# Breakthrough/PySceneDetect

Measured on NVIDIA H100. Metric: frames/sec scored (1080p, ContentDetector), higher is better.
Workload: dtype u8

## Files before the change

### pyscenedetect_b200/csrc/engine.cu

```cuda
#include <math.h>
#include <stdarg.h>
#include <string.h>

#include <vector>

#include "psd_common.cuh"

namespace psd {

static thread_local char g_err[512] = "";
std::atomic<uint64_t> g_launches{0};

void set_error(const char* fmt, ...) {
    va_list ap;
    va_start(ap, fmt);
    vsnprintf(g_err, sizeof(g_err), fmt, ap);
    va_end(ap);
}

static void build_taps(int src, int dst, std::vector<int32_t>& ofs, std::vector<int16_t>& coef) {
    ofs.resize(dst);
    coef.resize(2 * (size_t)dst);
    const double scale = (double)src / (double)dst;
    for (int d = 0; d < dst; ++d) {
// ... 161 lines not shown
    e->last_n = n;
    PSD_CUDA(cudaEventRecord(t1, st));
    e->ev_total.push_back({t0, t1});
    return PSD_OK;
}

extern "C" {

int psd_abi_version(void) { return PSD_ABI_VERSION; }
const char* psd_version(void) { return "psd_b200 0.1.0 (sm_90a)"; }
const char* psd_last_error(void) { return g_err; }
uint64_t psd_launch_count(void) { return g_launches.load(); }

int psd_device_count(void) {
    int n = 0;
    if (cudaGetDeviceCount(&n) != cudaSuccess) { cudaGetLastError(); return 0; }
    return n;
}

int psd_device_info(int device, char* name_out, size_t name_cap, int* cc_major, int* cc_minor,
                    int* sm_count, uint64_t* total_mem) {
    cudaDeviceProp p{};
    PSD_CUDA(cudaGetDeviceProperties(&p, device));
    if (name_out && name_cap) { strncpy(name_out, p.name, name_cap - 1); name_out[name_cap - 1] = 0; }
    if (cc_major) *cc_major = p.major;
    if (cc_minor) *cc_minor = p.minor;
    if (sm_count) *sm_count = p.multiProcessorCount;
    if (total_mem) *total_mem = (uint64_t)p.totalGlobalMem;
    return PSD_OK;
}

int psd_device_pci_bus_id(int device, char* out, size_t cap) {
    PSD_REQUIRE(out && cap >= 16, "psd_device_pci_bus_id: buffer too small");
    PSD_CUDA(cudaDeviceGetPCIBusId(out, (int)cap, device));
    return PSD_OK;
}

int psd_host_alloc(size_t bytes, void** out) {
    PSD_REQUIRE(out && bytes > 0, "psd_host_alloc: bad args");
    PSD_CUDA(cudaHostAlloc(out, bytes, cudaHostAllocDefault));
    return PSD_OK;
}
int psd_host_free(void* p) {
    if (p) PSD_CUDA(cudaFreeHost(p));
    return PSD_OK;
}
int psd_device_alloc(int device, size_t bytes, void** out) {
    PSD_REQUIRE(out && bytes > 0, "psd_device_alloc: bad args");
    PSD_CUDA(cudaSetDevice(device));
    PSD_CUDA(cudaMalloc(out, bytes));
    return PSD_OK;
}
int psd_device_free(int device, void* p) {
    PSD_CUDA(cudaSetDevice(device));
    if (p) PSD_CUDA(cudaFree(p));
    return PSD_OK;
}
int psd_memcpy_h2d(int device, void* dst, const void* src, size_t bytes) {
    PSD_CUDA(cudaSetDevice(device));
    PSD_CUDA(cudaMemcpy(dst, src, bytes, cudaMemcpyHostToDevice));
    return PSD_OK;
}
int psd_memcpy_d2h(int device, void* dst, const void* src, size_t bytes) {
    PSD_CUDA(cudaSetDevice(device));
    PSD_CUDA(cudaMemcpy(dst, src, bytes, cudaMemcpyDeviceToHost));
    return PSD_OK;
}

void psd_engine_destroy(psd_engine* e) {
    if (!e) return;
    cudaSetDevice(e->device);
    if (e->compute_stream) cudaStreamSynchronize(e->compute_stream);
    if (e->copy_stream) cudaStreamSynchronize(e->copy_stream);
    for (int s = 0; s < 2; ++s) {
        if (e->pinned[s]) cudaFreeHost(e->pinned[s]);
        if (e->dev_stage[s]) cudaFree(e->dev_stage[s]);
        if (e->slot_free[s]) cudaEventDestroy(e->slot_free[s]);
        if (e->h2d_done[s]) cudaEventDestroy(e->h2d_done[s]);
    }
    cudaFree(e->small); cudaFree(e->d_xofs); cudaFree(e->d_xa); cudaFree(e->d_yofs); cudaFree(e->d_ya);
    cudaFree(e->carry); cudaFree(e->d_sums); cudaFree(e->d_yhist); cudaFree(e->d_hash);
    hash_plan_destroy(&e->hash);
    cudaFree(e->eb.vplane); cudaFree(e->eb.vhist); cudaFree(e->eb.thresholds); cudaFree(e->eb.cand);
    cudaFree(e->eb.tmp); cudaFree(e->eb.bits_in); cudaFree(e->eb.bits_dil); cudaFree(e->eb.bits_hdil);
    cudaFree(e->eb.carry_bits); cudaFree(e->eb.dirty); cudaFree(e->eb.hyst_flags);
    for (cudaEvent_t ev : e->ev_pool) cudaEventDestroy(ev);
    if (e->copy_stream) cudaStreamDestroy(e->copy_stream);
    if (e->compute_stream) cudaStreamDestroy(e->compute_stream);
    delete e;
}

#define ENG_CUDA(expr)                                                                          \
    do {                                                                                        \
        cudaError_t _e = (expr);                                                                \
        if (_e != cudaSuccess) {                                                                \
            psd::set_error("%s failed: %s (%s:%d)", #expr, cudaGetErrorString(_e), __FILE__,    \
                           __LINE__);                                                           \
            psd_engine_destroy(e);                                                              \
            return (_e == cudaErrorMemoryAllocation) ? PSD_ERR_OOM : PSD_ERR_CUDA;              \
        }                                                                                       \
    } while (0)

int psd_engine_create(const psd_config* cfg, psd_engine** out) {
    PSD_REQUIRE(cfg && out, "psd_engine_create: null argument");
    PSD_REQUIRE(cfg->struct_size == (int32_t)sizeof(psd_config), "psd_config.struct_size mismatch");
    PSD_REQUIRE(cfg->src_width > 0 && cfg->src_height > 0 && cfg->width > 0 && cfg->height > 0,
                "frame sizes must be positive");
    PSD_REQUIRE((int64_t)cfg->src_width * cfg->src_height < (1LL << 30), "frame too large");
    PSD_REQUIRE(cfg->features != 0 && (cfg->features & ~31u) == 0, "bad feature mask 0x%x", cfg->features);
    PSD_REQUIRE(cfg->max_batch >= 1 && cfg->max_batch <= 4096, "max_batch must be in [1,4096]");
    PSD_REQUIRE(cfg->edge_kernel_size == 0 || (cfg->edge_kernel_size >= 3 && (cfg->edge_kernel_size & 1)),
                "kernel_size must be odd integer >= 3");
    PSD_REQUIRE(cfg->flags == 0, "psd_config.flags must be 0 (no flags are defined), got 0x%x", cfg->flags);
    int ndev = 0;
    if (cudaGetDeviceCount(&ndev) != cudaSuccess || ndev == 0) {
        cudaGetLastError();
        set_error("no CUDA device visible (this engine has no CPU fallback)");
        return PSD_ERR_NODEVICE;
    }
    PSD_REQUIRE(cfg->device >= 0 && cfg->device < ndev, "device %d out of range (%d visible)", cfg->device, ndev);
    cudaDeviceProp prop{};
    PSD_CUDA(cudaGetDeviceProperties(&prop, cfg->device));
    if (prop.major != 9 || prop.minor != 0) {
        set_error("device %d is sm_%d%d; this library is built for sm_90a only", cfg->device, prop.major,
                  prop.minor);
        return PSD_ERR_NODEVICE;
    }
    PSD_CUDA(cudaSetDevice(cfg->device));
    psd_engine* e = new (std::nothrow) psd_engine();
    if (!e) { set_error("out of host memory"); return PSD_ERR_OOM; }
    e->cfg = *cfg;
    e->device = cfg->device;
    e->sw = cfg->src_width; e->sh = cfg->src_height; e->W = cfg->width; e->H = cfg->height;
    e->resize = (e->sw != e->W) || (e->sh != e->H);
    e->P = (int64_t)e->W * e->H;
    e->frame_bytes = e->P * 3;
    e->small_stride = (e->frame_bytes + 15) & ~(int64_t)15;
    e->src_frame_bytes = (int64_t)e->sw * e->sh * 3;
    e->features = cfg->features | ((cfg->features & PSD_F_EDGES) ? PSD_F_HSV : 0);
    e->max_batch = cfg->max_batch;
    if (e->features & PSD_F_EDGES) {
        int k = cfg->edge_kernel_size;
        if (k == 0) {
            k = 4 + (int)nearbyint(sqrt((double)e->W * (double)e->H) / 192.0);
            if ((k & 1) == 0) k += 1;
        }
        if (edge_dilate_check(e->W, k) != PSD_OK) {
            psd_engine_destroy(e);
            return PSD_ERR_INVALID;
        }
        e->ksize = k;
    }
    if (e->features & PSD_F_HASH) {
        int rc = hash_plan_create(&e->hash, e->W, e->H, cfg->hash_size ? cfg->hash_size : 8,
                                  cfg->hash_lowpass ? cfg->hash_lowpass : 2, e->max_batch);
        if (rc) { psd_engine_destroy(e); return rc; }
    }
    ENG_CUDA(cudaStreamCreateWithFlags(&e->copy_stream, cudaStreamNonBlocking));
    ENG_CUDA(cudaStreamCreateWithFlags(&e->compute_stream, cudaStreamNonBlocking));
    for (int s = 0; s < 2; ++s) {
        ENG_CUDA(cudaEventCreateWithFlags(&e->slot_free[s], cudaEventDisableTiming));
        ENG_CUDA(cudaEventCreateWithFlags(&e->h2d_done[s], cudaEventDisableTiming));
    }
    ENG_CUDA(cudaMalloc(&e->carry, (size_t)e->frame_bytes));
    if (e->resize || e->frame_bytes % 16 != 0)
        ENG_CUDA(cudaMalloc(&e->small, (size_t)e->small_stride * e->max_batch));
    if (e->resize) {
        std::vector<int32_t> xo, yo; std::vector<int16_t> xa, ya;
        build_taps(e->sw, e->W, xo, xa);
        build_taps(e->sh, e->H, yo, ya);
        ENG_CUDA(cudaMalloc(&e->d_xofs, xo.size() * 4)); ENG_CUDA(cudaMalloc(&e->d_xa, xa.size() * 2));
        ENG_CUDA(cudaMalloc(&e->d_yofs, yo.size() * 4)); ENG_CUDA(cudaMalloc(&e->d_ya, ya.size() * 2));
        ENG_CUDA(cudaMemcpy(e->d_xofs, xo.data(), xo.size() * 4, cudaMemcpyHostToDevice));
        ENG_CUDA(cudaMemcpy(e->d_xa, xa.data(), xa.size() * 2, cudaMemcpyHostToDevice));
        ENG_CUDA(cudaMemcpy(e->d_yofs, yo.data(), yo.size() * 4, cudaMemcpyHostToDevice));
        ENG_CUDA(cudaMemcpy(e->d_ya, ya.data(), ya.size() * 2, cudaMemcpyHostToDevice));
    }
    if (e->features & PSD_F_EDGES) {
        const size_t plane = (size_t)e->P * e->max_batch;
        ENG_CUDA(cudaMalloc(&e->eb.vplane, plane));
        const size_t words = (size_t)e->H * ((e->W + 31) / 32);
        const size_t tiled = (size_t)edge_tile_words(e->W, e->H) * 4 * e->max_batch;
        ENG_CUDA(cudaMalloc(&e->eb.cand, tiled));
        ENG_CUDA(cudaMalloc(&e->eb.bits_in, tiled));
        ENG_CUDA(cudaMemset(e->eb.cand, 0, tiled));
        ENG_CUDA(cudaMemset(e->eb.bits_in, 0, tiled));
        ENG_CUDA(cudaMalloc(&e->eb.tmp, (size_t)e->P));
        ENG_CUDA(cudaMalloc(&e->eb.bits_dil, words * 4 * e->max_batch));
        if (edge_dilate_separable(e->ksize)) ENG_CUDA(cudaMalloc(&e->eb.bits_hdil, words * 4 * e->max_batch));
        ENG_CUDA(cudaMalloc(&e->eb.carry_bits, words * 4));
        ENG_CUDA(cudaMalloc(&e->eb.vhist, (size_t)e->max_batch * 256 * 4));
        ENG_CUDA(cudaMalloc(&e->eb.thresholds, (size_t)e->max_batch * 2 * 4));
        ENG_CUDA(cudaMalloc(&e->eb.hyst_flags, 64));
        const size_t n_tiles = (size_t)e->max_batch * ((e->W + 63) / 64) * ((e->H + 31) / 32);
        ENG_CUDA(cudaMalloc(&e->eb.dirty, 2 * n_tiles));
    }
    {
        int rc = ensure_capacity(e, 4096);
        if (rc) { psd_engine_destroy(e); return rc; }
    }
    *out = e;
    return PSD_OK;
}

int psd_engine_reset(psd_engine* e) {
    PSD_REQUIRE(e, "null engine");
    PSD_CUDA(cudaSetDevice(e->device));
    PSD_CUDA(cudaStreamSynchronize(e->copy_stream));
    PSD_CUDA(cudaStreamSynchronize(e->compute_stream));
    e->n_frames = 0;
    e->have_carry = false;
    e->halo_scored = false;
    e->last_n = 0;
    e->ev_next = 0; e->ev_score.clear(); e->ev_total.clear();
    return PSD_OK;
}

static int ensure_staging(psd_engine* e) {
    for (int s = 0; s < 2; ++s) {
        if (!e->dev_stage[s]) PSD_CUDA(cudaMalloc(&e->dev_stage[s], (size_t)e->src_frame_bytes * e->max_batch));
    }
    return PSD_OK;
}
static int ensure_pinned(psd_engine* e) {
    for (int s = 0; s < 2; ++s) {
        if (!e->pinned[s])
            PSD_CUDA(cudaHostAlloc((void**)&e->pinned[s], (size_t)e->src_frame_bytes * e->max_batch,
                                   cudaHostAllocDefault));
    }
    return PSD_OK;
}

static int stage_host(psd_engine* e, const uint8_t* bgr, int64_t n, int64_t frame_stride,
                      int64_t row_pitch, uint32_t flags, int slot) {
    const int64_t tight_row = (int64_t)e->sw * 3;
    PSD_CUDA(cudaEventSynchronize(e->slot_free[slot]));
    const uint8_t* src = bgr;
    int64_t fs = frame_stride, rp = row_pitch;
    if (!(flags & PSD_SUBMIT_PINNED)) {
        int rc = ensure_pinned(e);
        if (rc) return rc;
        uint8_t* dst = e->pinned[slot];
        if (rp == tight_row && fs == e->src_frame_bytes) {
            memcpy(dst, bgr, (size_t)(n * e->src_frame_bytes));
        } else {
            for (int64_t f = 0; f < n; ++f)
                for (int y = 0; y < e->sh; ++y)
                    memcpy(dst + f * e->src_frame_bytes + (int64_t)y * tight_row,
                           bgr + f * frame_stride + (int64_t)y * row_pitch, (size_t)tight_row);
        }
        src = dst; fs = e->src_frame_bytes; rp = tight_row;
    }
    if (rp == tight_row && fs == e->src_frame_bytes) {
        PSD_CUDA(cudaMemcpyAsync(e->dev_stage[slot], src, (size_t)(n * e->src_frame_bytes),
                                 cudaMemcpyHostToDevice, e->copy_stream));
    } else {
        for (int64_t f = 0; f < n; ++f)
            PSD_CUDA(cudaMemcpy2DAsync(e->dev_stage[slot] + f * e->src_frame_bytes, (size_t)tight_row,
                                       src + f * fs, (size_t)rp, (size_t)tight_row, (size_t)e->sh,
                                       cudaMemcpyHostToDevice, e->copy_stream));
    }
    PSD_CUDA(cudaEventRecord(e->h2d_done[slot], e->copy_stream));
    PSD_CUDA(cudaStreamWaitEvent(e->compute_stream, e->h2d_done[slot], 0));
    return PSD_OK;
}

int psd_engine_set_halo_device(psd_engine* e, const void* dptr) {
    PSD_REQUIRE(e && dptr, "psd_engine_set_halo_device: null argument");
    PSD_REQUIRE(e->n_frames == 0, "halo must be set before the first frame is submitted");
    PSD_CUDA(cudaSetDevice(e->device));
    e->have_carry = false;
    int rc = run_batch(e, (const uint8_t*)dptr, e->src_frame_bytes, 1, 0, true);
    if (rc) return rc;
    e->halo_scored = true;
    return PSD_OK;
}

int psd_engine_set_halo_host(psd_engine* e, const uint8_t* bgr, int64_t row_pitch) {
    PSD_REQUIRE(e && bgr, "psd_engine_set_halo_host: null argument");
    PSD_REQUIRE(e->n_frames == 0, "halo must be set before the first frame is submitted");
    PSD_REQUIRE(row_pitch >= (int64_t)e->sw * 3, "row_pitch smaller than a row");
    PSD_CUDA(cudaSetDevice(e->device));
    int rc = ensure_staging(e);
    if (rc) return rc;
    const int slot = e->next_slot;
    e->next_slot ^= 1;
    rc = stage_host(e, bgr, 1, row_pitch * e->sh, row_pitch, 0, slot);
    if (rc) return rc;
    rc = psd_engine_set_halo_device(e, e->dev_stage[slot]);
    if (rc) return rc;
    PSD_CUDA(cudaEventRecord(e->slot_free[slot], e->compute_stream));
    return PSD_OK;
}

int psd_engine_submit_device(psd_engine* e, const void* dptr, int64_t n, int64_t frame_stride) {
    PSD_REQUIRE(e && dptr, "psd_engine_submit_device: null argument");
    PSD_REQUIRE(n >= 0, "negative frame count");
    PSD_REQUIRE(frame_stride >= e->src_frame_bytes, "frame_stride smaller than a frame");
    if (n == 0) return PSD_OK;
    PSD_CUDA(cudaSetDevice(e->device));
    int rc = ensure_capacity(e, e->n_frames + n + 1);
    if (rc) return rc;
    const uint8_t* p = (const uint8_t*)dptr;
    int64_t done = 0;
    while (done < n) {
        const int64_t b = (n - done < e->max_batch) ? (n - done) : e->max_batch;
        rc = run_batch(e, p + done * frame_stride, frame_stride, b, e->n_frames + 1, false);
        if (rc) return rc;
        e->n_frames += b;
        done += b;
    }
    return PSD_OK;
}

int psd_engine_submit_host(psd_engine* e, const uint8_t* bgr, int64_t n, int64_t frame_stride,
                           int64_t row_pitch, uint32_t flags) {
    PSD_REQUIRE(e && bgr, "psd_engine_submit_host: null argument");
    PSD_REQUIRE(n >= 0, "negative frame count");
    PSD_REQUIRE(row_pitch >= (int64_t)e->sw * 3, "row_pitch smaller than a row");
    PSD_REQUIRE(n <= 1 || frame_stride >= (int64_t)e->sw * 3, "bad frame_stride");
    if (n == 0) return PSD_OK;
    PSD_CUDA(cudaSetDevice(e->device));
    int rc = ensure_staging(e);
    if (rc) return rc;
    rc = ensure_capacity(e, e->n_frames + n + 1);
    if (rc) return rc;
    int64_t done = 0;
    while (done < n) {
        const int64_t b = (n - done < e->max_batch) ? (n - done) : e->max_batch;
        const int slot = e->next_slot;
        e->next_slot ^= 1;
        rc = stage_host(e, bgr + done * frame_stride, b, frame_stride, row_pitch, flags, slot);
        if (rc) return rc;
        rc = run_batch(e, e->dev_stage[slot], e->src_frame_bytes, b, e->n_frames + 1, false);
        if (rc) return rc;
        PSD_CUDA(cudaEventRecord(e->slot_free[slot], e->compute_stream));
        e->n_frames += b;
        done += b;
    }
    return PSD_OK;
}

int psd_engine_sync(psd_engine* e) {
    PSD_REQUIRE(e, "null engine");
    PSD_CUDA(cudaSetDevice(e->device));
    PSD_CUDA(cudaStreamSynchronize(e->copy_stream));
    PSD_CUDA(cudaStreamSynchronize(e->compute_stream));
    return PSD_OK;
}

void* psd_engine_compute_stream(psd_engine* e) { return e ? (void*)e->compute_stream : nullptr; }
int64_t psd_engine_frame_count(const psd_engine* e) { return e ? e->n_frames : -1; }
int psd_engine_edge_kernel_size(const psd_engine* e) { return e ? e->ksize : -1; }

int psd_engine_read_sums(psd_engine* e, int64_t first, int64_t n, psd_frame_sums* out) {
    PSD_REQUIRE(e && out, "psd_engine_read_sums: null argument");
    PSD_REQUIRE(first >= -1 && n >= 0 && first + n <= e->n_frames, "frame range out of bounds");
    int rc = psd_engine_sync(e);
    if (rc) return rc;
    if (n) PSD_CUDA(cudaMemcpy(out, e->d_sums + first + 1, (size_t)n * sizeof(psd_frame_sums), cudaMemcpyDeviceToHost));
    return PSD_OK;
}

int psd_engine_read_yhist(psd_engine* e, int64_t first, int64_t n, uint32_t* out) {
    PSD_REQUIRE(e && out, "psd_engine_read_yhist: null argument");
    PSD_REQUIRE(e->features & PSD_F_YHIST, "engine was created without PSD_F_YHIST");
    PSD_REQUIRE(first >= -1 && n >= 0 && first + n <= e->n_frames, "frame range out of bounds");
    int rc = psd_engine_sync(e);
    if (rc) return rc;
    if (n) PSD_CUDA(cudaMemcpy(out, e->d_yhist + (first + 1) * 256, (size_t)n * 256 * 4, cudaMemcpyDeviceToHost));
    return PSD_OK;
}

int psd_engine_read_hash(psd_engine* e, int64_t first, int64_t n, uint64_t* out) {
    PSD_REQUIRE(e && out, "psd_engine_read_hash: null argument");
    PSD_REQUIRE(e->features & PSD_F_HASH, "engine was created without PSD_F_HASH");
    PSD_REQUIRE(first >= -1 && n >= 0 && first + n <= e->n_frames, "frame range out of bounds");
    int rc = psd_engine_sync(e);
    if (rc) return rc;
    if (n) PSD_CUDA(cudaMemcpy(out, e->d_hash + (first + 1) * e->hash.words, (size_t)n * e->hash.words * 8, cudaMemcpyDeviceToHost));
    return PSD_OK;
}

int psd_engine_device_hash(psd_engine* e, const uint64_t** hashes) {
    PSD_REQUIRE(e && hashes, "psd_engine_device_hash: null argument");
    *hashes = e->d_hash ? e->d_hash + e->hash.words : nullptr;
    return PSD_OK;
}

int psd_engine_device_results(psd_engine* e, const psd_frame_sums** sums, const uint32_t** yhist) {
    PSD_REQUIRE(e, "null engine");
    if (sums) *sums = e->d_sums + 1;
    if (yhist) *yhist = e->d_yhist ? e->d_yhist + 256 : nullptr;
    return PSD_OK;
}

int psd_engine_timing_reset(psd_engine* e) {
    PSD_REQUIRE(e, "null engine");
    int rc = psd_engine_sync(e);
    if (rc) return rc;
    e->ev_next = 0; e->ev_score.clear(); e->ev_total.clear();
    return PSD_OK;
}

int psd_engine_timing_ms(psd_engine* e, float* total_ms, float* score_ms, uint64_t* score_launches) {
    PSD_REQUIRE(e, "null engine");
    int rc = psd_engine_sync(e);
    if (rc) return rc;
    float tot = 0.f, sc = 0.f;
    for (auto& p : e->ev_total) { float ms = 0; PSD_CUDA(cudaEventElapsedTime(&ms, p.first, p.second)); tot += ms; }
    for (auto& p : e->ev_score) { float ms = 0; PSD_CUDA(cudaEventElapsedTime(&ms, p.first, p.second)); sc += ms; }
    if (total_ms) *total_ms = tot;
    if (score_ms) *score_ms = sc;
    if (score_launches) *score_launches = e->ev_score.size();
    return PSD_OK;
}

int psd_engine_debug_plane(psd_engine* e, int which, int64_t index, uint8_t* out, size_t cap) {
    PSD_REQUIRE(e && out, "psd_engine_debug_plane: null argument");
    PSD_REQUIRE(index >= 0 && index < e->last_n, "index outside the last batch");
    int rc = psd_engine_sync(e);
    if (rc) return rc;
    if (which == 0) {
        PSD_REQUIRE(cap >= (size_t)e->frame_bytes, "buffer too small");
        PSD_CUDA(cudaMemcpy(out, e->last_scored + index * e->last_scored_stride, (size_t)e->frame_bytes, cudaMemcpyDeviceToHost));
        return PSD_OK;
    }
    PSD_REQUIRE(e->features & PSD_F_EDGES, "engine was created without PSD_F_EDGES");
    PSD_REQUIRE(cap >= (size_t)e->P, "buffer too small");
    PSD_REQUIRE(which >= 1 && which <= 3, "unknown plane %d", which);
    if (which == 2 || which == 3) {
        const size_t words = (size_t)e->H * ((e->W + 31) / 32);
        const uint32_t* bits = which == 3 ? e->eb.bits_dil + index * words
                                          : e->eb.bits_in + index * (size_t)edge_tile_words(e->W, e->H);
        rc = edge_unpack(bits, e->eb.tmp, e->W, e->H, which == 2, e->compute_stream);
        if (rc) return rc;
        PSD_CUDA(cudaStreamSynchronize(e->compute_stream));
        PSD_CUDA(cudaMemcpy(out, e->eb.tmp, (size_t)e->P, cudaMemcpyDeviceToHost));
        return PSD_OK;
    }
    PSD_CUDA(cudaMemcpy(out, e->eb.vplane + index * e->P, (size_t)e->P, cudaMemcpyDeviceToHost));
    return PSD_OK;
}

static int scan_to_host(psd_engine* e, double* d_tmp, double* out, size_t count) {
    PSD_CUDA(cudaStreamSynchronize(e->compute_stream));
    PSD_CUDA(cudaMemcpy(out, d_tmp, count * sizeof(double), cudaMemcpyDeviceToHost));
    return PSD_OK;
}

int psd_engine_scan_content_host(psd_engine* e, int64_t first, int64_t n, const double weights[4],
                                 double weight_abs_sum, double* out_components, double* out_content_val) {
    PSD_REQUIRE(e && weights && out_content_val, "psd_engine_scan_content_host: null argument");
    PSD_REQUIRE(first >= 0 && n >= 0 && first + n <= e->n_frames, "frame range out of bounds");
    if (n == 0) return PSD_OK;
    PSD_CUDA(cudaSetDevice(e->device));
    double* tmp = nullptr;
    PSD_CUDA(cudaMalloc(&tmp, (size_t)n * 5 * sizeof(double)));
    int rc = psd_scan_content(e->d_sums + 1 + first, n, e->P, weights, weight_abs_sum, tmp + n, tmp, e->compute_stream);
    if (!rc) rc = scan_to_host(e, tmp, out_content_val, (size_t)n);
    if (!rc && out_components) rc = scan_to_host(e, tmp + n, out_components, (size_t)n * 4);
    cudaFree(tmp);
    return rc;
}

int psd_engine_scan_adaptive_host(psd_engine* e, const double* scores_host, int64_t n, int32_t window_width,
                                  double min_content_val, double* out_ratio) {
    PSD_REQUIRE(e && scores_host && out_ratio && n >= 0, "psd_engine_scan_adaptive_host: bad argument");
    if (n == 0) return PSD_OK;
    PSD_CUDA(cudaSetDevice(e->device));
    double* tmp = nullptr;
    PSD_CUDA(cudaMalloc(&tmp, (size_t)n * 2 * sizeof(double)));
    int rc = PSD_OK;
    if (cudaMemcpyAsync(tmp, scores_host, (size_t)n * sizeof(double), cudaMemcpyHostToDevice, e->compute_stream) != cudaSuccess) {
        set_error("scores upload failed"); rc = PSD_ERR_CUDA;
    }
    if (!rc) rc = psd_scan_adaptive(tmp, n, window_width, min_content_val, tmp + n, e->compute_stream);
    if (!rc) rc = scan_to_host(e, tmp + n, out_ratio, (size_t)n);
    cudaFree(tmp);
    return rc;
}

int psd_engine_scan_average_host(psd_engine* e, int64_t first, int64_t n, double* out_avg) {
    PSD_REQUIRE(e && out_avg, "psd_engine_scan_average_host: null argument");
    PSD_REQUIRE(first >= 0 && n >= 0 && first + n <= e->n_frames, "frame range out of bounds");
    if (n == 0) return PSD_OK;
    PSD_CUDA(cudaSetDevice(e->device));
    double* tmp = nullptr;
    PSD_CUDA(cudaMalloc(&tmp, (size_t)n * sizeof(double)));
    int rc = psd_scan_average(e->d_sums + 1 + first, n, e->P * 3, tmp, e->compute_stream);
    if (!rc) rc = scan_to_host(e, tmp, out_avg, (size_t)n);
    cudaFree(tmp);
    return rc;
}

int psd_engine_scan_hist_correl_host(psd_engine* e, int64_t first, int64_t n, int32_t bins, double* out) {
    PSD_REQUIRE(e && out, "psd_engine_scan_hist_correl_host: null argument");
    PSD_REQUIRE(e->features & PSD_F_YHIST, "engine was created without PSD_F_YHIST");
    PSD_REQUIRE(first >= 0 && n >= 0 && first + n <= e->n_frames, "frame range out of bounds");
    if (n == 0) return PSD_OK;
    PSD_CUDA(cudaSetDevice(e->device));
    double* tmp = nullptr;
    PSD_CUDA(cudaMalloc(&tmp, (size_t)n * sizeof(double)));
    const uint32_t* prev = (first > 0 || e->halo_scored) ? e->d_yhist + first * 256 : nullptr;
    int rc = psd_scan_hist_correl(e->d_yhist + (first + 1) * 256, n, bins, prev, tmp, e->compute_stream);
    if (!rc) rc = scan_to_host(e, tmp, out, (size_t)n);
    cudaFree(tmp);
    return rc;
}

int psd_scan_hash_dist(const uint64_t* hashes, int64_t n, int32_t hash_size, const uint64_t* prev_hash, double* out,
                       void* stream) {
    PSD_REQUIRE(hashes && out && n >= 0 && hash_size >= 1 && hash_size <= 32768, "psd_scan_hash_dist: bad arguments");
    return launch_hash_dist(hashes, n, hash_size, prev_hash, out, (cudaStream_t)stream);
}

int psd_engine_scan_hash_dist_host(psd_engine* e, int64_t first, int64_t n, double* out) {
    PSD_REQUIRE(e && out, "psd_engine_scan_hash_dist_host: null argument");
    PSD_REQUIRE(e->features & PSD_F_HASH, "engine was created without PSD_F_HASH");
    PSD_REQUIRE(first >= 0 && n >= 0 && first + n <= e->n_frames, "frame range out of bounds");
    if (n == 0) return PSD_OK;
    PSD_CUDA(cudaSetDevice(e->device));
    double* tmp = nullptr;
    PSD_CUDA(cudaMalloc(&tmp, (size_t)n * sizeof(double)));
    const uint64_t* prev = (first > 0 || e->halo_scored) ? e->d_hash + first * e->hash.words : nullptr;
    int rc = psd_scan_hash_dist(e->d_hash + (first + 1) * e->hash.words, n, e->hash.size, prev, tmp, e->compute_stream);
    if (!rc) rc = scan_to_host(e, tmp, out, (size_t)n);
    cudaFree(tmp);
    return rc;
}

int psd_synth_frames(int device, void* d_out, const int32_t* params_host, int64_t n, int32_t width,
                     int32_t height, int64_t frame_stride, void* stream) {
    PSD_REQUIRE(d_out && params_host && n > 0 && width > 0 && height > 0, "psd_synth_frames: bad args");
    PSD_REQUIRE(frame_stride >= (int64_t)width * height * 3, "frame_stride smaller than a frame");
    PSD_CUDA(cudaSetDevice(device));
    int32_t* d_params = nullptr;
    PSD_CUDA(cudaMalloc(&d_params, (size_t)n * 24 * 4));
    PSD_CUDA(cudaMemcpy(d_params, params_host, (size_t)n * 24 * 4, cudaMemcpyHostToDevice));
    int rc = PSD_OK;
    int64_t done = 0;
    while (!rc && done < n) {
        const int64_t b = (n - done < 4096) ? (n - done) : 4096;
        rc = launch_synth((uint8_t*)d_out + done * frame_stride, d_params + done * 24, b, width, height,
                          frame_stride, (cudaStream_t)stream);
        done += b;
    }
    if (!rc && cudaStreamSynchronize((cudaStream_t)stream) != cudaSuccess) { set_error("synth sync failed: %s", cudaGetErrorString(cudaGetLastError())); rc = PSD_ERR_CUDA; }
    cudaFree(d_params);
    return rc;
}

}
```

### pyscenedetect_b200/csrc/score_kernel.cu

```cuda
#include "hsv_half2.cuh"
#include "psd_common.cuh"

namespace psd {

constexpr int kPxPerThread = 16;

__device__ __forceinline__ uint32_t smem_u32(const void* p) {
    return (uint32_t)__cvta_generic_to_shared(p);
}
__device__ __forceinline__ void mbar_init(unsigned long long* bar, uint32_t count) {
    asm volatile("mbarrier.init.shared::cta.b64 [%0], %1;" ::"r"(smem_u32(bar)), "r"(count));
}
__device__ __forceinline__ void mbar_expect_tx(unsigned long long* bar, uint32_t bytes) {
    asm volatile("mbarrier.arrive.expect_tx.shared::cta.b64 _, [%0], %1;" ::"r"(smem_u32(bar)),
                 "r"(bytes)
                 : "memory");
}
__device__ __forceinline__ void bulk_g2s(void* dst, const void* src, uint32_t bytes,
                                         unsigned long long* bar) {
    asm volatile(
        "cp.async.bulk.shared::cluster.global.mbarrier::complete_tx::bytes [%0], [%1], %2, [%3];" ::
            "r"(smem_u32(dst)),
        "l"(src), "r"(bytes), "r"(smem_u32(bar))
        : "memory");
}

constexpr int kWsConsumerWarps = 24;
constexpr int kWsConsumers = kWsConsumerWarps * 32;
constexpr int kWsThreads = kWsConsumers + 32;
constexpr int kWsStages = 4;
constexpr int kWsUnroll = 4;
constexpr int kWsStripPx = kWsConsumers * kPxPerThread;
constexpr int kWsStripBytes = kWsStripPx * 3;
static_assert(kWsStages % kWsUnroll == 0, "the stage ring must be a whole number of loop bodies");

struct __align__(128) WsSmem {
    uint8_t ring[kWsStages][kWsStripBytes];
    float lut[256 * 64];
    unsigned long long full[kWsStages];
    unsigned long long empty[kWsStages];
    uint32_t accl[kWsStages][4][32];
    uint32_t accl_seen[kWsStages][4][32];
    uint32_t accl_sink[kWsStages][4][32];
    uint32_t yhist[kWsStages][256];
    uint32_t vhist[kWsStages][256];
};

__device__ __forceinline__ uint32_t sad4_acc(uint32_t a, uint32_t b, uint32_t c) {
    uint32_t r;
    asm volatile("vabsdiff4.u32.u32.u32.add %0, %1, %2, %3;" : "=r"(r) : "r"(a), "r"(b), "r"(c));
    return r;
}
template <int OFF>
__device__ __forceinline__ void mbar_wait_hint_off(uint32_t bar, uint32_t parity) {
    asm volatile(
        "{\n\t"
        ".reg .pred p;\n\t"
        "WAIT_%=:\n\t"
        "mbarrier.try_wait.parity.shared::cta.b64 p, [%0+%3], %1, %2;\n\t"
        "@p bra DONE_%=;\n\t"
        "bra WAIT_%=;\n\t"
        "DONE_%=:\n\t"
        "}" ::"r"(bar),
        "r"(parity), "r"(20000u), "n"(OFF)
        : "memory");
}
__device__ __forceinline__ void mbar_wait_hint(unsigned long long* bar, uint32_t parity) {
    mbar_wait_hint_off<0>(smem_u32(bar), parity);
}
template <int OFF>
__device__ __forceinline__ void lds128_off(uint32_t addr, uint32_t& x, uint32_t& y, uint32_t& z, uint32_t& w) {
    asm volatile("ld.shared.v4.u32 {%0,%1,%2,%3}, [%4+%5];" : "=r"(x), "=r"(y), "=r"(z), "=r"(w) : "r"(addr), "n"(OFF));
}
template <int OFF>
__device__ __forceinline__ void red_shared_add_off(uint32_t addr, uint32_t v) {
    asm volatile("red.shared.add.u32 [%0+%2], %1;" ::"r"(addr), "r"(v), "n"(OFF) : "memory");
}
template <int OFF>
__device__ __forceinline__ void mbar_arrive_off(uint32_t bar) {
    asm volatile("mbarrier.arrive.shared::cta.b64 _, [%0+%1];" ::"r"(bar), "n"(OFF) : "memory");
}

__host__ __device__ __forceinline__ int chunk_first(int c, int n_frames, int n_chunks) {
    return (int)(((long long)c * n_frames) / n_chunks);
}
struct WsItem {
    int f0, nf;
    int px0, valid_px;
    int it_begin;
    int slots;
    int walked;
};
__device__ __forceinline__ WsItem ws_item(const ScoreArgs& a, int item) {
    WsItem w;
    const int chunk = item % a.n_chunks;
    const int strip = item / a.n_chunks;
    w.f0 = chunk_first(chunk, a.n_frames, a.n_chunks);
    w.nf = chunk_first(chunk + 1, a.n_frames, a.n_chunks) - w.f0;
    w.px0 = strip * kWsStripPx;
    w.valid_px = min(kWsStripPx, a.n_pixels - w.px0) & ~15;
    const bool have_halo = (a.features & PSD_F_HSV) && (w.f0 > 0 || a.prev != nullptr);
    w.it_begin = have_halo ? 0 : 1;
    w.walked = w.nf + 1 - w.it_begin;
    w.slots = (w.walked + kWsUnroll - 1) / kWsUnroll * kWsUnroll;
    return w;
}

struct WsAddr {
    uint32_t ring;
    uint32_t full;
    uint32_t acc;
};

template <uint32_t F, int J>
__device__ __forceinline__ void ws_step(const ScoreArgs& a, WsSmem& sm, const WsAddr& ad, uint32_t parity, int stage0,
                                        uint32_t sad_acc, bool mine, int fi, int my_px, int lane, uint32_t zero,
                                        const LutView7& lut7, const Px16& prev, Px16& cur) {
    constexpr bool kHSV = (F & PSD_F_HSV) != 0;
    constexpr bool kSUM = (F & PSD_F_BGRSUM) != 0;
    constexpr bool kYH = (F & PSD_F_YHIST) != 0;
    constexpr bool kEDGE = (F & PSD_F_EDGES) != 0;
    if (kHSV) {
        if ((J & 1) == 0) {
            mbar_wait_hint_off<J * 8>(ad.full, parity);
            mbar_wait_hint_off<J * 8 + 8>(ad.full, parity);
        }
    } else {
        mbar_wait_hint_off<J * 8>(ad.full, parity);
    }
    uint32_t w[12];
    lds128_off<J * kWsStripBytes>(ad.ring, w[0], w[1], w[2], w[3]);
    lds128_off<J * kWsStripBytes + 16>(ad.ring, w[4], w[5], w[6], w[7]);
    lds128_off<J * kWsStripBytes + 32>(ad.ring, w[8], w[9], w[10], w[11]);
    if (kHSV) {
        hsv16_v7(w, cur, lut7);
        uint32_t sad_h = sad4_acc(cur.h[0], prev.h[0], zero), sad_s = sad4_acc(cur.s[0], prev.s[0], zero),
                 sad_v = sad4_acc(cur.v[0], prev.v[0], zero);
#pragma unroll
        for (int j = 1; j < 4; ++j) {
            sad_h = sad4_acc(cur.h[j], prev.h[j], sad_h);
            sad_s = sad4_acc(cur.s[j], prev.s[j], sad_s);
            sad_v = sad4_acc(cur.v[j], prev.v[j], sad_v);
        }
        red_shared_add_off<J * 512>(sad_acc, sad_h);
        red_shared_add_off<J * 512 + 128>(sad_acc, sad_s);
        red_shared_add_off<J * 512 + 256>(sad_acc, sad_v);
        if (kEDGE && mine) {
            uint8_t* vp = a.vplane + (int64_t)fi * a.n_pixels + my_px;
            if ((a.n_pixels & 15) == 0) {
                *reinterpret_cast<uint4*>(vp) = make_uint4(cur.v[0], cur.v[1], cur.v[2], cur.v[3]);
            } else {
                for (int p = 0; p < kPxPerThread; ++p) vp[p] = (uint8_t)(cur.v[p >> 2] >> ((p & 3) * 8));
            }
            const uint32_t vh = smem_u32(sm.vhist[stage0 + J]);
#pragma unroll
            for (int p = 0; p < kPxPerThread; ++p)
                red_shared_add_off<0>(__dp4a(cur.v[p >> 2], 4u << ((p & 3) * 8), vh), 1u);
        }
    }
    if (mine) {
        if (kSUM) {
            uint32_t bsum = 0;
#pragma unroll
            for (int j = 0; j < 12; ++j) bsum = __dp4a(w[j], 0x01010101u, bsum);
            red_shared_add_off<J * 512 + 384>(ad.acc, bsum);
        }
        if (kYH) {
            uint32_t* hist = sm.yhist[stage0 + J];
#define PSD_YH(i) atomicAdd(&hist[y_of_pixel<i>(w)], 1u);
            PSD_YH(0) PSD_YH(1) PSD_YH(2) PSD_YH(3) PSD_YH(4) PSD_YH(5) PSD_YH(6) PSD_YH(7)
            PSD_YH(8) PSD_YH(9) PSD_YH(10) PSD_YH(11) PSD_YH(12) PSD_YH(13) PSD_YH(14) PSD_YH(15)
#undef PSD_YH
        }
    }
    if (lane == 0) mbar_arrive_off<kWsStages * 8 + J * 8>(ad.full);
}

template <int J>
__device__ __forceinline__ void ws_null_step(const WsAddr& ad, uint32_t parity, int lane) {
    mbar_wait_hint_off<J * 8>(ad.full, parity);
    if (lane == 0) mbar_arrive_off<kWsStages * 8 + J * 8>(ad.full);
}

template <uint32_t F>
__global__ void __launch_bounds__(kWsThreads, 1) psd_score_ws_kernel(const ScoreArgs a) {
    extern __shared__ __align__(128) uint8_t smem_raw[];
    WsSmem& sm = *reinterpret_cast<WsSmem*>(smem_raw);
    constexpr bool kHSV = (F & PSD_F_HSV) != 0;
    constexpr bool kSUM = (F & PSD_F_BGRSUM) != 0;
    constexpr bool kYH = (F & PSD_F_YHIST) != 0;
    constexpr bool kEDGE = (F & PSD_F_EDGES) != 0;
    constexpr int U = kWsUnroll;

    const int tid = threadIdx.x;
    const int lane = tid & 31;
    const int n_items = a.n_chunks * a.n_strips;

    for (int i = tid; i < kWsStages * 256; i += kWsThreads) {
        (&sm.yhist[0][0])[i] = 0;
        (&sm.vhist[0][0])[i] = 0;
    }
    for (int i = tid; i < kWsStages * 4 * 32; i += kWsThreads) {
        (&sm.accl[0][0][0])[i] = 0;
        (&sm.accl_seen[0][0][0])[i] = 0;
        (&sm.accl_sink[0][0][0])[i] = 0;
    }
    if (kHSV) lut_fill7(sm.lut, tid, kWsThreads);
    if (tid == 0) {
        for (int s = 0; s < kWsStages; ++s) {
            mbar_init(&sm.full[s], 1);
            mbar_init(&sm.empty[s], kWsConsumerWarps);
        }
        asm volatile("fence.mbarrier_init.release.cluster;" ::: "memory");
    }
    __syncthreads();

    if (tid >= kWsConsumers) {
        struct Cursor {
            int item, slot;
            WsItem w;
        };
        auto load = [&](Cursor& c) { if (c.item < n_items) c.w = ws_item(a, c.item); };
        auto advance = [&](Cursor& c) {
            if (++c.slot == c.w.slots) { c.slot = 0; c.item += gridDim.x; load(c); }
        };
        auto issue = [&](const Cursor& c, int stage) {
            if (c.slot < c.w.walked) {
                const int fi = c.w.f0 - 1 + c.w.it_begin + c.slot;
                const uint8_t* src = (fi < 0 ? a.prev : a.frames + (int64_t)fi * a.frame_stride) + (int64_t)c.w.px0 * 3;
                const uint32_t bytes = (uint32_t)c.w.valid_px * 3u;
                mbar_expect_tx(&sm.full[stage], bytes);
                bulk_g2s(sm.ring[stage], src, bytes, &sm.full[stage]);
            } else {
                mbar_arrive_off<0>(smem_u32(&sm.full[stage]));
            }
        };
        Cursor iss{(int)blockIdx.x, 0, {}}, ret{(int)blockIdx.x, 0, {}};
        load(iss);
        ret.w = iss.w;
        for (int s = 0; s < kWsStages && iss.item < n_items; ++s) {
            if (lane == 0) issue(iss, s);
            advance(iss);
        }
        int stage = 0;
        uint32_t parity = 0;
        while (ret.item < n_items) {
            mbar_wait_hint(&sm.empty[stage], parity);
            const int it = ret.w.it_begin + ret.slot;
            const bool real = ret.slot < ret.w.walked;
            const bool own = real && it >= 1;
            const int fi = ret.w.f0 - 1 + it;
            uint32_t tot[4] = {0u, 0u, 0u, 0u};
            if (own && (kHSV || kSUM)) {
#pragma unroll
                for (int c = 0; c < 4; ++c)
                    if ((c < 3 && kHSV) || (c == 3 && kSUM)) tot[c] = sm.accl[stage][c][lane];
            }
            if (own) {
                if (kYH) {
#pragma unroll
                    for (int b = lane; b < 256; b += 32) {
                        const uint32_t v = sm.yhist[stage][b];
                        if (v) { sm.yhist[stage][b] = 0; atomicAdd(&a.yhist[(int64_t)fi * 256 + b], v); }
                    }
                }
                if (kEDGE) {
#pragma unroll
                    for (int b = lane; b < 256; b += 32) {
                        const uint32_t v = sm.vhist[stage][b];
                        if (v) { sm.vhist[stage][b] = 0; atomicAdd(&a.vhist[(int64_t)fi * 256 + b], v); }
                    }
                }
                if (ret.item < a.n_chunks && lane == 0)
                    a.sums[fi].has_prev = (fi > 0 || a.prev != nullptr) ? 1ull : 0ull;
            }
            __syncwarp();
            if (iss.item < n_items) {
                if (lane == 0) issue(iss, stage);
                advance(iss);
            }
            if (own && (kHSV || kSUM)) {
#pragma unroll
                for (int c = 0; c < 4; ++c) {
                    if ((c < 3 && !kHSV) || (c == 3 && !kSUM)) continue;
                    const uint32_t d = tot[c] - sm.accl_seen[stage][c][lane];
                    sm.accl_seen[stage][c][lane] = tot[c];
                    const uint32_t v = __reduce_add_sync(0xFFFFFFFFu, d);
                    if (lane == 0 && v)
                        atomicAdd(reinterpret_cast<unsigned long long*>(&a.sums[fi]) + (c < 3 ? c : 4),
                                  (unsigned long long)v);
                }
            }
            advance(ret);
            if (++stage == kWsStages) { stage = 0; parity ^= 1u; }
        }
        return;
    }

    const LutView7 lut7 = make_lut7(smem_u32(sm.lut), lane);
    const uint32_t zero = a.shift24 ^ 0x01000000u;
    const uint32_t ring0 = smem_u32(sm.ring[0]) + tid * 48;
    const uint32_t full0 = smem_u32(&sm.full[0]);
    const uint32_t accl0 = smem_u32(&sm.accl[0][0][lane]);
    const uint32_t sink0 = smem_u32(&sm.accl_sink[0][0][lane]);
    int stage0 = 0;
    uint32_t parity = 0;
    WsAddr ad{ring0, full0, 0u};
    auto next_body = [&](uint32_t acc0) {
        stage0 += U;
        if (stage0 == kWsStages) {
            stage0 = 0;
            parity ^= 1u;
            ad.ring = ring0; ad.full = full0; ad.acc = acc0;
        } else {
            ad.ring += U * kWsStripBytes; ad.full += U * 8; ad.acc += U * 512;
        }
    };
    for (int item = blockIdx.x; item < n_items; item += gridDim.x) {
        const WsItem wi = ws_item(a, item);
        const int my_px = wi.px0 + tid * kPxPerThread;
        const bool active = tid * kPxPerThread < wi.valid_px;
        const uint32_t acc0 = active ? accl0 : sink0;
        ad.acc = acc0 + stage0 * 512;
        Px16 P0, P1;
#pragma unroll
        for (int j = 0; j < 4; ++j) P0.h[j] = P0.s[j] = P0.v[j] = P1.h[j] = P1.s[j] = P1.v[j] = 0;
        const int n = wi.walked;
        const int fbase = wi.f0 - 1 + wi.it_begin;
        int k = 0;
        uint32_t acc_first = sink0 + stage0 * 512;
#pragma unroll 1
        for (; k + U <= n; k += U) {
            const bool first_mine = active && (wi.it_begin + k >= 1);
            ws_step<F, 0>(a, sm, ad, parity, stage0, acc_first, first_mine, fbase + k, my_px, lane, zero, lut7, P0, P1);
            ws_step<F, 1>(a, sm, ad, parity, stage0, ad.acc, active, fbase + k + 1, my_px, lane, zero, lut7, P1, P0);
            ws_step<F, 2>(a, sm, ad, parity, stage0, ad.acc, active, fbase + k + 2, my_px, lane, zero, lut7, P0, P1);
            ws_step<F, 3>(a, sm, ad, parity, stage0, ad.acc, active, fbase + k + 3, my_px, lane, zero, lut7, P1, P0);
            next_body(acc0);
            acc_first = ad.acc;
        }
        if (k < n) {
            const int r = n - k;
            ws_step<F, 0>(a, sm, ad, parity, stage0, acc_first, active && (wi.it_begin + k >= 1), fbase + k, my_px,
                              lane, zero, lut7, P0, P1);
            if (r > 1) ws_step<F, 1>(a, sm, ad, parity, stage0, ad.acc, active, fbase + k + 1, my_px, lane, zero, lut7, P1, P0);
            else ws_null_step<1>(ad, parity, lane);
            if (r > 2) ws_step<F, 2>(a, sm, ad, parity, stage0, ad.acc, active, fbase + k + 2, my_px, lane, zero, lut7, P0, P1);
            else ws_null_step<2>(ad, parity, lane);
            ws_null_step<3>(ad, parity, lane);
            next_body(acc0);
        }
    }
}

static int pick_chunks(int n_frames, int n_strips, int grid) {
    long long best_cost = -1;
    int best = 1;
    const int c_max = n_frames < 4096 ? n_frames : 4096;
    for (int c = 1; c <= c_max; ++c) {
        const int longest = (n_frames + c - 1) / c;
        if (longest < 8 && c > 1) break;
        const long long per_cta = ((long long)n_strips * c + grid - 1) / grid;
        const long long cost = per_cta * (longest + 1);
        if (best_cost < 0 || cost < best_cost) { best_cost = cost; best = c; }
    }
    return best;
}

template <uint32_t F>
static int launch_ws(ScoreArgs a, int n_ws_strips, cudaStream_t stream) {
    const int smem = (int)sizeof(WsSmem);
    static int sm_count = 0;
    if (sm_count == 0) {
        int dev = 0;
        PSD_CUDA(cudaGetDevice(&dev));
        PSD_CUDA(cudaDeviceGetAttribute(&sm_count, cudaDevAttrMultiProcessorCount, dev));
    }
    PSD_CUDA(cudaFuncSetAttribute(psd_score_ws_kernel<F>, cudaFuncAttributeMaxDynamicSharedMemorySize, smem));
    a.shift24 = 0x01000000u;
    a.features = F;
    a.n_strips = n_ws_strips;
    a.n_chunks = pick_chunks(a.n_frames, n_ws_strips, sm_count);
    if (a.n_chunks > a.n_frames) a.n_chunks = a.n_frames;
    const int64_t items = (int64_t)a.n_chunks * n_ws_strips;
    PSD_REQUIRE(items > 0 && items < 2147483647LL, "score work items out of range (%lld)", (long long)items);
    const int grid = (int)(items < sm_count ? items : sm_count);
    psd_score_ws_kernel<F><<<grid, kWsThreads, smem, stream>>>(a);
    PSD_CHECK_LAUNCH();
    count_launch();
    return PSD_OK;
}

static int dispatch_ws(const ScoreArgs& a, uint32_t f, int n_ws_strips, cudaStream_t s) {
    switch (f & 15u) {
#define CASE(F) case F: return launch_ws<F>(a, n_ws_strips, s);
        CASE(1) CASE(2) CASE(3) CASE(4) CASE(5) CASE(6) CASE(7)
        CASE(9) CASE(11) CASE(13) CASE(15)
#undef CASE
        default:
            set_error("unsupported feature mask 0x%x", f);
            return PSD_ERR_INVALID;
    }
}

constexpr int kTailThreads = 128;
constexpr int kLutBytes = 256 * 64 * 4;

__device__ __forceinline__ void load_tail(const uint8_t* src, int n_bytes, uint32_t (&w)[12]) {
#pragma unroll
    for (int j = 0; j < 12; ++j) w[j] = 0;
#pragma unroll
    for (int k = 0; k < 48; ++k)
        if (k < n_bytes) w[k >> 2] |= (uint32_t)src[k] << ((k & 3) * 8);
}

__global__ void __launch_bounds__(kTailThreads) psd_score_tail_kernel(const ScoreArgs a) {
    extern __shared__ __align__(128) float lut[];
    const bool hsv = (a.features & PSD_F_HSV) != 0;
    if (hsv) lut_fill7(lut, threadIdx.x, blockDim.x);
    __syncthreads();
    const int fi = blockIdx.x * blockDim.x + threadIdx.x;
    if (fi >= a.n_frames) return;
    const int p16 = a.n_pixels & ~15, n = a.n_pixels - p16;
    const uint8_t* prev = fi > 0 ? a.frames + (int64_t)(fi - 1) * a.frame_stride : a.prev;
    uint32_t w[12];
    load_tail(a.frames + (int64_t)fi * a.frame_stride + (int64_t)p16 * 3, 3 * n, w);
    unsigned long long* sums = reinterpret_cast<unsigned long long*>(&a.sums[fi]);
    if (hsv) {
        const LutView7 lut7 = make_lut7(smem_u32(lut), threadIdx.x & 31);
        Px16 cur;
        hsv16_v7(w, cur, lut7);
        if (prev) {
            uint32_t wp[12];
            load_tail(prev + (int64_t)p16 * 3, 3 * n, wp);
            Px16 pre;
            hsv16_v7(wp, pre, lut7);
            uint32_t sad_h = 0, sad_s = 0, sad_v = 0;
#pragma unroll
            for (int j = 0; j < 4; ++j) {
                sad_h = __vsadu4(cur.h[j], pre.h[j]) + sad_h;
                sad_s = __vsadu4(cur.s[j], pre.s[j]) + sad_s;
                sad_v = __vsadu4(cur.v[j], pre.v[j]) + sad_v;
            }
            atomicAdd(sums + 0, (unsigned long long)sad_h);
            atomicAdd(sums + 1, (unsigned long long)sad_s);
            atomicAdd(sums + 2, (unsigned long long)sad_v);
        }
        if (a.features & PSD_F_EDGES) {
            uint8_t* vp = a.vplane + (int64_t)fi * a.n_pixels + p16;
            for (int p = 0; p < n; ++p) {
                const uint32_t v = (cur.v[p >> 2] >> ((p & 3) * 8)) & 0xFFu;
                vp[p] = (uint8_t)v;
                atomicAdd(&a.vhist[(int64_t)fi * 256 + v], 1u);
            }
        }
    }
    if (a.features & PSD_F_BGRSUM) {
        uint32_t bsum = 0;
#pragma unroll
        for (int j = 0; j < 12; ++j) bsum = __dp4a(w[j], 0x01010101u, bsum);
        atomicAdd(sums + 4, (unsigned long long)bsum);
    }
    if (a.features & PSD_F_YHIST) {
        for (int p = 0; p < n; ++p)
            atomicAdd(&a.yhist[(int64_t)fi * 256 + y_px(byte_of(w, 3 * p), byte_of(w, 3 * p + 1), byte_of(w, 3 * p + 2))],
                      1u);
    }
    if (p16 == 0) a.sums[fi].has_prev = (fi > 0 || a.prev != nullptr) ? 1ull : 0ull;
}

static int launch_tail(ScoreArgs a, uint32_t features, cudaStream_t stream) {
    PSD_CUDA(cudaFuncSetAttribute(psd_score_tail_kernel, cudaFuncAttributeMaxDynamicSharedMemorySize, kLutBytes));
    a.features = features;
    const int grid = (a.n_frames + kTailThreads - 1) / kTailThreads;
    psd_score_tail_kernel<<<grid, kTailThreads, (features & PSD_F_HSV) ? kLutBytes : 0, stream>>>(a);
    PSD_CHECK_LAUNCH();
    count_launch();
    return PSD_OK;
}

int launch_score(const ScoreArgs& a, uint32_t features, cudaStream_t stream) {
    if (features & PSD_F_EDGES) features |= PSD_F_HSV;
    PSD_REQUIRE(a.n_frames > 0 && a.n_pixels > 0, "empty score launch");
    const uintptr_t al = reinterpret_cast<uintptr_t>(a.frames) | (uintptr_t)a.frame_stride |
                         reinterpret_cast<uintptr_t>(a.prev);
    PSD_REQUIRE((al & 15) == 0, "score pass input is not 16-byte aligned");
    const int p16 = a.n_pixels & ~15;
    if (p16 > 0) {
        const int rc = dispatch_ws(a, features, (p16 + kWsStripPx - 1) / kWsStripPx, stream);
        if (rc) return rc;
    }
    if (p16 < a.n_pixels) return launch_tail(a, features, stream);
    return PSD_OK;
}

__global__ void psd_test_hsv_kernel(const uint8_t* bgr, int64_t n_groups, uint8_t* h, uint8_t* s,
                                    uint8_t* v, uint8_t* y) {
    extern __shared__ __align__(128) float lutmem[];
    lut_fill7(lutmem, threadIdx.x, blockDim.x);
    const LutView7 lut7 = make_lut7(smem_u32(lutmem), threadIdx.x & 31);
    __syncthreads();
    for (int64_t g = blockIdx.x * (int64_t)blockDim.x + threadIdx.x; g < n_groups;
         g += (int64_t)gridDim.x * blockDim.x) {
        uint32_t w[12];
        const uint4* p = reinterpret_cast<const uint4*>(bgr + g * 48);
        const uint4 q0 = p[0], q1 = p[1], q2 = p[2];
        w[0] = q0.x; w[1] = q0.y; w[2] = q0.z; w[3] = q0.w;
        w[4] = q1.x; w[5] = q1.y; w[6] = q1.z; w[7] = q1.w;
        w[8] = q2.x; w[9] = q2.y; w[10] = q2.z; w[11] = q2.w;
        Px16 o;
        hsv16_v7(w, o, lut7);
        *reinterpret_cast<uint4*>(h + g * 16) = make_uint4(o.h[0], o.h[1], o.h[2], o.h[3]);
        *reinterpret_cast<uint4*>(s + g * 16) = make_uint4(o.s[0], o.s[1], o.s[2], o.s[3]);
        *reinterpret_cast<uint4*>(v + g * 16) = make_uint4(o.v[0], o.v[1], o.v[2], o.v[3]);
        for (int px = 0; px < 16; ++px)
            y[g * 16 + px] = (uint8_t)y_px(byte_of(w, 3 * px), byte_of(w, 3 * px + 1), byte_of(w, 3 * px + 2));
    }
}

}

extern "C" int psd_test_hsv(int device, const uint8_t* bgr_host, int64_t n_pixels, uint8_t* h_out,
                            uint8_t* s_out, uint8_t* v_out, uint8_t* y_out) {
    using namespace psd;
    PSD_REQUIRE(n_pixels > 0 && (n_pixels % 16) == 0, "n_pixels must be a positive multiple of 16");
    PSD_CUDA(cudaSetDevice(device));
    int sm_count = 0;
    PSD_CUDA(cudaDeviceGetAttribute(&sm_count, cudaDevAttrMultiProcessorCount, device));
    uint8_t *d_bgr = nullptr, *d_out = nullptr;
    PSD_CUDA(cudaMalloc(&d_bgr, (size_t)n_pixels * 3));
    PSD_CUDA(cudaMalloc(&d_out, (size_t)n_pixels * 4));
    PSD_CUDA(cudaMemcpy(d_bgr, bgr_host, (size_t)n_pixels * 3, cudaMemcpyHostToDevice));
    uint8_t* dh = d_out;
    uint8_t* ds = d_out + n_pixels;
    uint8_t* dv = d_out + 2 * n_pixels;
    uint8_t* dy = d_out + 3 * n_pixels;
    PSD_CUDA(cudaFuncSetAttribute(psd_test_hsv_kernel, cudaFuncAttributeMaxDynamicSharedMemorySize, kLutBytes));
    psd_test_hsv_kernel<<<sm_count * 2, 256, kLutBytes>>>(d_bgr, n_pixels / 16, dh, ds, dv, dy);
    PSD_CHECK_LAUNCH();
    count_launch();
    PSD_CUDA(cudaDeviceSynchronize());
    PSD_CUDA(cudaMemcpy(h_out, dh, (size_t)n_pixels, cudaMemcpyDeviceToHost));
    PSD_CUDA(cudaMemcpy(s_out, ds, (size_t)n_pixels, cudaMemcpyDeviceToHost));
    PSD_CUDA(cudaMemcpy(v_out, dv, (size_t)n_pixels, cudaMemcpyDeviceToHost));
    PSD_CUDA(cudaMemcpy(y_out, dy, (size_t)n_pixels, cudaMemcpyDeviceToHost));
    cudaFree(d_bgr);
    cudaFree(d_out);
    return PSD_OK;
}
```

Baseline: 343,400.

## Use one producer warp per ring stage and process device input in a single batch

The single producer warp, which handled TMA issue and per-stage flush for all four stages in sequence, becomes four side warps, one per stage and SM sub-partition. Each warp issues bulk copies and drains accumulators for its own stage. Accumulators are zeroed on read instead of being diffed against a seen copy, which drops the accl_seen array. Device submissions with aligned pointers, no resize, and no edge or hash features now run as one large batch, which removes per-batch launch overhead. The extra warps raise the block's thread count, and the zero-on-read scheme depends on consumers not writing between the read and the reset.

```diff
diff --git a/pyscenedetect_b200/csrc/engine.cu b/pyscenedetect_b200/csrc/engine.cu
--- a/pyscenedetect_b200/csrc/engine.cu
+++ b/pyscenedetect_b200/csrc/engine.cu
@@ -487,9 +487,12 @@
     int rc = ensure_capacity(e, e->n_frames + n + 1);
     if (rc) return rc;
     const uint8_t* p = (const uint8_t*)dptr;
+    const bool in_place = !e->resize && !(e->features & (PSD_F_EDGES | PSD_F_HASH)) &&
+                          (((uintptr_t)p | (uintptr_t)frame_stride) & 15) == 0;
+    const int64_t batch = in_place ? ((int64_t)1 << 30) : (int64_t)e->max_batch;
     int64_t done = 0;
     while (done < n) {
-        const int64_t b = (n - done < e->max_batch) ? (n - done) : e->max_batch;
+        const int64_t b = (n - done < batch) ? (n - done) : batch;
         rc = run_batch(e, p + done * frame_stride, frame_stride, b, e->n_frames + 1, false);
         if (rc) return rc;
         e->n_frames += b;
diff --git a/pyscenedetect_b200/csrc/score_kernel.cu b/pyscenedetect_b200/csrc/score_kernel.cu
--- a/pyscenedetect_b200/csrc/score_kernel.cu
+++ b/pyscenedetect_b200/csrc/score_kernel.cu
@@ -27,8 +27,10 @@
 
 constexpr int kWsConsumerWarps = 24;
 constexpr int kWsConsumers = kWsConsumerWarps * 32;
-constexpr int kWsThreads = kWsConsumers + 32;
 constexpr int kWsStages = 4;
+constexpr int kWsSideWarps = kWsStages;
+constexpr int kWsThreads = kWsConsumers + kWsSideWarps * 32;
+static_assert(kWsSideWarps == 4 && kWsConsumerWarps % 4 == 0, "one side warp per SM sub-partition");
 constexpr int kWsUnroll = 4;
 constexpr int kWsStripPx = kWsConsumers * kPxPerThread;
 constexpr int kWsStripBytes = kWsStripPx * 3;
@@ -40,7 +42,6 @@
     unsigned long long full[kWsStages];
     unsigned long long empty[kWsStages];
     uint32_t accl[kWsStages][4][32];
-    uint32_t accl_seen[kWsStages][4][32];
     uint32_t accl_sink[kWsStages][4][32];
     uint32_t yhist[kWsStages][256];
     uint32_t vhist[kWsStages][256];
@@ -202,7 +203,6 @@
     }
     for (int i = tid; i < kWsStages * 4 * 32; i += kWsThreads) {
         (&sm.accl[0][0][0])[i] = 0;
-        (&sm.accl_seen[0][0][0])[i] = 0;
         (&sm.accl_sink[0][0][0])[i] = 0;
     }
     if (kHSV) lut_fill7(sm.lut, tid, kWsThreads);
@@ -220,32 +220,33 @@
             int item, slot;
             WsItem w;
         };
+        const int rs = (tid - kWsConsumers) >> 5;
         auto load = [&](Cursor& c) { if (c.item < n_items) c.w = ws_item(a, c.item); };
         auto advance = [&](Cursor& c) {
-            if (++c.slot == c.w.slots) { c.slot = 0; c.item += gridDim.x; load(c); }
+            c.slot += kWsStages;
+            if (c.slot >= c.w.slots) { c.slot = rs; c.item += gridDim.x; load(c); }
         };
-        auto issue = [&](const Cursor& c, int stage) {
-            if (c.slot < c.w.walked) {
-                const int fi = c.w.f0 - 1 + c.w.it_begin + c.slot;
-                const uint8_t* src = (fi < 0 ? a.prev : a.frames + (int64_t)fi * a.frame_stride) + (int64_t)c.w.px0 * 3;
-                const uint32_t bytes = (uint32_t)c.w.valid_px * 3u;
-                mbar_expect_tx(&sm.full[stage], bytes);
-                bulk_g2s(sm.ring[stage], src, bytes, &sm.full[stage]);
-            } else {
-                mbar_arrive_off<0>(smem_u32(&sm.full[stage]));
-            }
+        auto issue = [&](Cursor& c) {
+            if (lane == 0) {
+                if (c.slot < c.w.walked) {
+                    const int fi = c.w.f0 - 1 + c.w.it_begin + c.slot;
+                    const uint8_t* src = (fi < 0 ? a.prev : a.frames + (int64_t)fi * a.frame_stride) + (int64_t)c.w.px0 * 3;
+                    const uint32_t bytes = (uint32_t)c.w.valid_px * 3u;
+                    mbar_expect_tx(&sm.full[rs], bytes);
+                    bulk_g2s(sm.ring[rs], src, bytes, &sm.full[rs]);
+                } else {
+                    mbar_arrive_off<0>(smem_u32(&sm.full[rs]));
+                }
+            }
+            advance(c);
         };
-        Cursor iss{(int)blockIdx.x, 0, {}}, ret{(int)blockIdx.x, 0, {}};
-        load(iss);
-        ret.w = iss.w;
-        for (int s = 0; s < kWsStages && iss.item < n_items; ++s) {
-            if (lane == 0) issue(iss, s);
-            advance(iss);
-        }
-        int stage = 0;
+        Cursor ret{(int)blockIdx.x, rs, {}};
+        load(ret);
+        Cursor iss = ret;
+        issue(iss);
         uint32_t parity = 0;
         while (ret.item < n_items) {
-            mbar_wait_hint(&sm.empty[stage], parity);
+            mbar_wait_hint(&sm.empty[rs], parity);
             const int it = ret.w.it_begin + ret.slot;
             const bool real = ret.slot < ret.w.walked;
             const bool own = real && it >= 1;
@@ -253,46 +254,45 @@
             uint32_t tot[4] = {0u, 0u, 0u, 0u};
             if (own && (kHSV || kSUM)) {
 #pragma unroll
-                for (int c = 0; c < 4; ++c)
-                    if ((c < 3 && kHSV) || (c == 3 && kSUM)) tot[c] = sm.accl[stage][c][lane];
+                for (int c = 0; c < 4; ++c) {
+                    if ((c < 3 && kHSV) || (c == 3 && kSUM)) {
+                        tot[c] = sm.accl[rs][c][lane];
+                        sm.accl[rs][c][lane] = 0;
+                    }
+                }
             }
             if (own) {
                 if (kYH) {
 #pragma unroll
                     for (int b = lane; b < 256; b += 32) {
-                        const uint32_t v = sm.yhist[stage][b];
-                        if (v) { sm.yhist[stage][b] = 0; atomicAdd(&a.yhist[(int64_t)fi * 256 + b], v); }
+                        const uint32_t v = sm.yhist[rs][b];
+                        if (v) { sm.yhist[rs][b] = 0; atomicAdd(&a.yhist[(int64_t)fi * 256 + b], v); }
                     }
                 }
                 if (kEDGE) {
 #pragma unroll
                     for (int b = lane; b < 256; b += 32) {
-                        const uint32_t v = sm.vhist[stage][b];
-                        if (v) { sm.vhist[stage][b] = 0; atomicAdd(&a.vhist[(int64_t)fi * 256 + b], v); }
+                        const uint32_t v = sm.vhist[rs][b];
+                        if (v) { sm.vhist[rs][b] = 0; atomicAdd(&a.vhist[(int64_t)fi * 256 + b], v); }
                     }
                 }
                 if (ret.item < a.n_chunks && lane == 0)
                     a.sums[fi].has_prev = (fi > 0 || a.prev != nullptr) ? 1ull : 0ull;
             }
             __syncwarp();
-            if (iss.item < n_items) {
-                if (lane == 0) issue(iss, stage);
-                advance(iss);
-            }
+            if (iss.item < n_items) issue(iss);
             if (own && (kHSV || kSUM)) {
 #pragma unroll
                 for (int c = 0; c < 4; ++c) {
                     if ((c < 3 && !kHSV) || (c == 3 && !kSUM)) continue;
-                    const uint32_t d = tot[c] - sm.accl_seen[stage][c][lane];
-                    sm.accl_seen[stage][c][lane] = tot[c];
-                    const uint32_t v = __reduce_add_sync(0xFFFFFFFFu, d);
+                    const uint32_t v = __reduce_add_sync(0xFFFFFFFFu, tot[c]);
                     if (lane == 0 && v)
                         atomicAdd(reinterpret_cast<unsigned long long*>(&a.sums[fi]) + (c < 3 ? c : 4),
                                   (unsigned long long)v);
                 }
             }
             advance(ret);
-            if (++stage == kWsStages) { stage = 0; parity ^= 1u; }
+            parity ^= 1u;
         }
         return;
     }
```

Result: faster. 361,300 (median of 6 runs) (+5.2%).
